# shiyao-li/NextBestPath

Hardware: AMD Instinct MI355X
Metric: exploration steps/s (+ NBP maps/s) at 256x256 (higher is better)
Workload: dtype f32

## Files before the change

### include/nbp_hip.h

```cpp
#ifndef NBP_HIP_H
#define NBP_HIP_H

#include <stddef.h>
#include <stdint.h>

#ifdef __cplusplus
extern "C" {
#endif

#define NBP_E_ARG      (-1)
#define NBP_E_WS       (-2)
#define NBP_E_SHAPE    (-3)

int nbp_abi_version(void);
int nbp_device_info(char* arch_host, int arch_len, int* cu_count_host);
int nbp_tuning_active(void);
int nbp_tuning_report(char* buf_host, int len);
int nbp_tile_kernel_symbol(int tile, char* buf_host, int len);

#define NBP_N_CONV 48

typedef struct nbp_weights nbp_weights;

size_t nbp_packed_weights_bytes(void);
// ... 47 lines not shown
int nbp_pack_conv_weight_split(const float* w_oihw, int N, int C, int ksize, const float* scale_or_null, int c_off,
                               int c_total, void* dst_planes, void* wamax_out, void* stream);
int nbp_amax_f32(const float* x, long long n, void* amax_inout, void* stream);
int nbp_pack_upconv_weight_split(const float* w_oihw, int N, int C, void* dst_planes, void* wamax_out, void* stream);
int nbp_upconv3x3_split_f32(const float* src, int C, int B, int H, int W, const void* planes_up, const void* wamax_up, int N,
                            const float* scale, const float* shift, int relu, float* out, const void* amax_in_or_null,
                            void* amax_out_or_null, int split_k, void* ws, size_t ws_bytes, void* stream);
size_t nbp_conv_split_workspace_bytes(int B, int H, int W, int N, int split_k);
size_t nbp_conv_split_planned_workspace_bytes(int B, int H, int W, int C, int N, int ups, int* split_k_out);
size_t nbp_conv_split_planned_workspace_bytes_k(int B, int H, int W, int C, int N, int ups, int split_k, int* split_k_out);
int nbp_conv3x3_split_f32(const float* src0, int C0, const float* src1, int C1, int ups, int B, int H, int W,
                          const void* w_planes, const void* wamax, int N, const float* scale, const float* shift, int relu,
                          float* out, const void* amax_in_or_null, void* amax_out_or_null, int split_k, void* ws,
                          size_t ws_bytes, void* stream);
size_t nbp_conv_first_wgrad_workspace_bytes(void);
int nbp_conv_first_wgrad_f32(const float* x_nchw, int B, int H, int W, const float* dy, float* dw, void* ws, size_t ws_bytes, void* stream);
int nbp_prepack_weights_split(const void* descs_dev, int n, void* wamax_words, void* stream);
int nbp_prepack_desc_bytes(void);
int nbp_pack_conv_weight_split_prezeroed(const float* w_oihw, int N, int C, int ksize, int c_total, void* dst_planes,
                                         void* wamax_zeroed, void* stream);
int nbp_pack_conv_weight_split_dgrad_known(const float* w_oihw, int N, int C, int c_total, void* dst_planes, const void* wamax_known,
                                           void* stream);
int nbp_pack_upconv_weight_split_dgrad(const float* w_oihw, int N, int C, void* dst_planes, void* wamax_out, void* stream);
size_t nbp_upconv_split_dgrad_workspace_bytes(int B, int H, int W, int N, int C);
int nbp_upconv3x3_split_dgrad_f32(const float* dy, int N, int B, int H, int W, const void* planes, const void* wamax, int C,
                                  const float* scale, const float* shift, float* dx, const void* amax_in, void* amax_out_or_null,
                                  void* ws, size_t ws_bytes, void* stream);
size_t nbp_upconv_wgrad_split_workspace_bytes(int B, int Hs, int Ws, int C, int N);
int nbp_upconv_wgrad_split_f32(const float* x, int C, int B, int Hs, int Ws, const float* dy, int N, float* dw,
                               const void* amax_x, const void* amax_y, void* ws, size_t ws_bytes, void* stream);
int nbp_conv1x1_split_f32(const float* src, int C, long long M, const void* w_planes, const void* wamax, int N,
                          const float* scale, const float* shift, int relu, float* out, const void* amax_in, void* stream);
int nbp_pack_conv1x1_weight_split_dgrad(const float* w_nc, int N, int C, void* dst_planes, void* wamax_out, void* stream);
int nbp_pack_conv_weight_split_dgrad(const float* w_oihw, int N, int C, int c_total, void* dst_planes, void* wamax_out, void* stream);

int nbp_conv_bn_part_rows(int B, int H, int W);
int nbp_conv3x3_split_bn_f32(const float* src0, int C0, const float* src1, int C1, int ups, int B, int H, int W,
                             const void* w_planes, const void* wamax, int N, const float* scale, const float* shift, int relu,
                             float* out, const void* amax_in_or_null, void* amax_out_or_null, int split_k, void* ws,
                             size_t ws_bytes, double* bn_part, int* bn_rows, void* stream);
int nbp_upconv3x3_split_bn_f32(const float* src, int C, int B, int H, int W, const void* planes_up, const void* wamax_up, int N,
                               const float* scale, const float* shift, int relu, float* out, const void* amax_in_or_null,
                               void* amax_out_or_null, int split_k, void* ws, size_t ws_bytes, double* bn_part, int* bn_rows,
                               void* stream);
int nbp_pack_conv_weight_split_h1(const float* w_oihw, int N, int C, int ksize, const float* scale_or_null, int c_off,
                                  int c_total, void* dst_planes, void* wamax_out, void* stream);
int nbp_pack_conv_weight_split_prezeroed_h1(const float* w_oihw, int N, int C, int ksize, int c_total, void* dst_planes,
                                            void* wamax_zeroed, void* stream);
int nbp_pack_conv_weight_split_dgrad_h1(const float* w_oihw, int N, int C, int c_total, void* dst_planes, void* wamax_out, void* stream);
int nbp_pack_conv_weight_split_dgrad_known_h1(const float* w_oihw, int N, int C, int c_total, void* dst_planes, const void* wamax_known,
                                              void* stream);
int nbp_pack_upconv_weight_split_h1(const float* w_oihw, int N, int C, void* dst_planes, void* wamax_out, void* stream);
int nbp_pack_upconv_weight_split_dgrad_h1(const float* w_oihw, int N, int C, void* dst_planes, void* wamax_out, void* stream);
int nbp_pack_conv1x1_weight_split_dgrad_h1(const float* w_nc, int N, int C, void* dst_planes, void* wamax_out, void* stream);
int nbp_prepack_weights_split_h1(const void* descs_dev, int n, void* wamax_words, void* stream);
int nbp_conv3x3_split_f32_h1(const float* src0, int C0, const float* src1, int C1, int ups, int B, int H, int W,
                             const void* w_planes, const void* wamax, int N, const float* scale, const float* shift, int relu,
                             float* out, const void* amax_in_or_null, void* amax_out_or_null, int split_k, void* ws,
                             size_t ws_bytes, void* stream);
int nbp_conv3x3_split_bn_f32_h1(const float* src0, int C0, const float* src1, int C1, int ups, int B, int H, int W,
                                const void* w_planes, const void* wamax, int N, const float* scale, const float* shift, int relu,
                                float* out, const void* amax_in_or_null, void* amax_out_or_null, int split_k, void* ws,
                                size_t ws_bytes, double* bn_part, int* bn_rows, void* stream);
int nbp_upconv3x3_split_f32_h1(const float* src, int C, int B, int H, int W, const void* planes_up, const void* wamax_up, int N,
                               const float* scale, const float* shift, int relu, float* out, const void* amax_in_or_null,
                               void* amax_out_or_null, int split_k, void* ws, size_t ws_bytes, void* stream);
// ... 352 lines not shown
```

### nextbestpath_amd/_lib.py

```python
from __future__ import annotations

import ctypes as C
import os
import threading

HERE = os.path.dirname(os.path.abspath(__file__))
LIB_PATH = os.path.join(HERE, "libnbp_hip.so")

_vp, _i, _ll, _f, _sz, _d = C.c_void_p, C.c_int, C.c_longlong, C.c_float, C.c_size_t, C.c_double

SIGNATURES = {
    "nbp_abi_version": (_i, []),
    "nbp_device_info": (_i, [C.c_char_p, _i, C.POINTER(_i)]),
    "nbp_tuning_active": (_i, []),
    "nbp_tuning_report": (_i, [C.c_char_p, _i]),
    "nbp_tile_kernel_symbol": (_i, [_i, C.c_char_p, _i]),
    "nbp_packed_weights_bytes": (_sz, []),
    "nbp_pack_weights": (_i, [C.POINTER(_vp), C.POINTER(_vp), C.POINTER(_vp), _vp, _sz, _vp, C.POINTER(_vp)]),
    "nbp_free_weights": (None, [_vp]),
    "nbp_forward_workspace_bytes": (_sz, [_i, _i]),
    "nbp_forward_f32": (_i, [_vp, _vp, _i, _i, _vp, _vp, _vp, _sz, _vp]),
    "nbp_forward_flops": (_d, [_i, _i]),
    "nbp_conv_igemm_f32": (_i, [_vp, _i, _vp, _i, _i, _i, _i, _i, _i, _vp, _i, _vp, _vp, _i, _vp, _i, _i, _vp,
                                _sz, _vp]),
# ... 87 lines not shown
SIGNATURES["nbp_packed_weights_bytes_bf16"] = SIGNATURES["nbp_packed_weights_bytes"]
SIGNATURES["nbp_pack_upconv_weight_bf16"] = (_i, [_vp, _i, _i, _vp, _vp])
SIGNATURES["nbp_forward_workspace_bytes_bf16"] = SIGNATURES["nbp_forward_workspace_bytes"]
SIGNATURES["nbp_forward_bf16"] = SIGNATURES["nbp_forward_f32"]
SIGNATURES["nbp_packed_weights_bytes_split"] = SIGNATURES["nbp_packed_weights_bytes"]
SIGNATURES["nbp_pack_weights_split"] = SIGNATURES["nbp_pack_weights"]
SIGNATURES["nbp_forward_workspace_bytes_split"] = SIGNATURES["nbp_forward_workspace_bytes"]
SIGNATURES["nbp_forward_split_f32"] = SIGNATURES["nbp_forward_f32"]
SIGNATURES["nbp_forward_timed_split_f32"] = SIGNATURES["nbp_forward_timed_f32"]
SIGNATURES["nbp_pack_conv_weight_split"] = (_i, [_vp, _i, _i, _i, _vp, _i, _i, _vp, _vp, _vp])
SIGNATURES["nbp_amax_f32"] = (_i, [_vp, _ll, _vp, _vp])
SIGNATURES["nbp_pack_upconv_weight_split"] = (_i, [_vp, _i, _i, _vp, _vp, _vp])
SIGNATURES["nbp_upconv3x3_split_f32"] = (_i, [_vp, _i, _i, _i, _i, _vp, _vp, _i, _vp, _vp, _i, _vp, _vp, _vp, _i, _vp, _sz, _vp])
SIGNATURES["nbp_conv_split_workspace_bytes"] = SIGNATURES["nbp_conv_igemm_workspace_bytes"]
SIGNATURES["nbp_conv_split_planned_workspace_bytes"] = (_sz, [_i, _i, _i, _i, _i, _i, _vp])
SIGNATURES["nbp_conv_split_planned_workspace_bytes_k"] = (_sz, [_i, _i, _i, _i, _i, _i, _i, _vp])
SIGNATURES["nbp_conv3x3_split_f32"] = (_i, [_vp, _i, _vp, _i, _i, _i, _i, _i, _vp, _vp, _i, _vp, _vp, _i, _vp, _vp, _vp, _i, _vp,
                                            _sz, _vp])
SIGNATURES["nbp_pack_upconv_weight_split_dgrad"] = (_i, [_vp, _i, _i, _vp, _vp, _vp])
SIGNATURES["nbp_upconv_split_dgrad_workspace_bytes"] = (_sz, [_i, _i, _i, _i, _i])
SIGNATURES["nbp_upconv3x3_split_dgrad_f32"] = (_i, [_vp, _i, _i, _i, _i, _vp, _vp, _i, _vp, _vp, _vp, _vp, _vp, _vp, _sz, _vp])
SIGNATURES["nbp_upconv_wgrad_split_workspace_bytes"] = (_sz, [_i, _i, _i, _i, _i])
SIGNATURES["nbp_upconv_wgrad_split_f32"] = (_i, [_vp, _i, _i, _i, _i, _vp, _i, _vp, _vp, _vp, _vp, _sz, _vp])
SIGNATURES["nbp_pack_conv_weight_split_prezeroed"] = (_i, [_vp, _i, _i, _i, _i, _vp, _vp, _vp])
SIGNATURES["nbp_pack_conv_weight_split_dgrad_known"] = (_i, [_vp, _i, _i, _i, _vp, _vp, _vp])
SIGNATURES["nbp_prepack_weights_split"] = (_i, [_vp, _i, _vp, _vp])
SIGNATURES["nbp_prepack_desc_bytes"] = (_i, [])
SIGNATURES["nbp_rowscale_amax_f32"] = (_i, [_vp, _vp, _ll, _i, _vp, _vp, _vp])
SIGNATURES["nbp_conv_first_linear_f32"] = (_i, [_vp, _i, _i, _i, _vp, _vp, _vp, _vp, _vp])
SIGNATURES["nbp_conv_first_wgrad_workspace_bytes"] = (_sz, [])
SIGNATURES["nbp_conv_first_wgrad_f32"] = (_i, [_vp, _i, _i, _i, _vp, _vp, _vp, _sz, _vp])
SIGNATURES["nbp_conv1x1_split_f32"] = (_i, [_vp, _i, _ll, _vp, _vp, _i, _vp, _vp, _i, _vp, _vp, _vp])
SIGNATURES["nbp_pack_conv1x1_weight_split_dgrad"] = (_i, [_vp, _i, _i, _vp, _vp, _vp])
SIGNATURES["nbp_pack_conv_weight_split_dgrad"] = (_i, [_vp, _i, _i, _i, _vp, _vp, _vp])
SIGNATURES["nbp_conv_bn_part_rows"] = (_i, [_i, _i, _i])
SIGNATURES["nbp_conv3x3_split_bn_f32"] = (_i, [_vp, _i, _vp, _i, _i, _i, _i, _i, _vp, _vp, _i, _vp, _vp, _i, _vp, _vp, _vp, _i, _vp,
                                               _sz, _vp, C.POINTER(_i), _vp])
SIGNATURES["nbp_upconv3x3_split_bn_f32"] = (_i, [_vp, _i, _i, _i, _i, _vp, _vp, _i, _vp, _vp, _i, _vp, _vp, _vp, _i, _vp, _sz, _vp,
                                                 C.POINTER(_i), _vp])
SIGNATURES["nbp_bn_train_forward_part4_f32"] = (_i, [_vp, _ll, _i, _vp, _vp, _f, _f, _vp, _vp, _i, _vp, _vp, _vp, _vp, _vp, _i, _vp, _i, _vp, _vp])
for _n in ("nbp_pack_conv_weight_split", "nbp_pack_conv_weight_split_prezeroed", "nbp_pack_conv_weight_split_dgrad",
           "nbp_pack_conv_weight_split_dgrad_known", "nbp_pack_upconv_weight_split", "nbp_pack_upconv_weight_split_dgrad",
           "nbp_pack_conv1x1_weight_split_dgrad", "nbp_prepack_weights_split", "nbp_conv3x3_split_f32", "nbp_conv3x3_split_bn_f32",
           "nbp_upconv3x3_split_f32", "nbp_upconv3x3_split_bn_f32", "nbp_upconv3x3_split_dgrad_f32", "nbp_conv1x1_split_f32",
           "nbp_upconv_wgrad_split_f32", "nbp_conv_wgrad_split_f32"):
    SIGNATURES[_n + "_h1"] = SIGNATURES[_n]
SIGNATURES["nbp_conv_igemm_bf16"] = SIGNATURES["nbp_conv_igemm_f32"]
SIGNATURES["nbp_conv_igemm_bf16_workspace_bytes"] = SIGNATURES["nbp_conv_igemm_workspace_bytes"]
SIGNATURES["nbp_pack_conv_weight_bf16"] = SIGNATURES["nbp_pack_conv_weight"]
SIGNATURES["nbp_f32_to_bf16"] = (_i, [_vp, _ll, _vp, _vp])
SIGNATURES["nbp_bf16_to_f32"] = (_i, [_vp, _ll, _vp, _vp])
_fpp, _ipp = C.POINTER(_f), C.POINTER(_i)
SIGNATURES["nbp_scene_fill_workspace_bytes"] = (_sz, [_fpp, _ipp, _i, _ll, _d])
SIGNATURES["nbp_scene_fill_cells_f32"] = (_i, [_vp, _ll, _vp, _fpp, _ipp, _i, _d, _i, C.c_uint, _vp, _vp, _vp, _sz, _vp])
SIGNATURES["nbp_scene_gather_f32"] = (_i, [_vp, _vp, _i, _i, _vp, _ll, _vp, _vp])
SIGNATURES["nbp_scene_coverage_workspace_bytes"] = (_sz, [_fpp, _ipp, _i, _d])
SIGNATURES["nbp_scene_coverage_f32"] = (_i, [_vp, _vp, _i, _vp, _vp, _i, _fpp, _ipp, _d, _vp, _vp, _sz, _vp])
SIGNATURES["nbp_coverage_plan_bytes"] = (_sz, [_fpp, _fpp, _f, _i])
SIGNATURES["nbp_coverage_plan_workspace_bytes"] = (_sz, [_fpp, _fpp, _f, _i])
SIGNATURES["nbp_coverage_plan_build_f32"] = (_i, [_vp, _i, _f, _fpp, _fpp, _vp, _sz, _vp, _sz, _vp])
SIGNATURES["nbp_coverage_count_planned_f32"] = (_i, [_vp, _i, _f, _fpp, _fpp, _vp, _ll, _vp, _ll, C.c_uint, C.c_uint, _vp, _vp,
                                                     _vp])
SIGNATURES["nbp_points_in_fov_u8"] = (_i, [_vp, _i, _fpp, _i, _i, _i, _f, _f, _vp, _vp, _vp])
SIGNATURES["nbp_sample_points_f32"] = (_i, [_vp, _ll, _vp, _ll, C.c_uint, _vp, _vp, _vp])
SIGNATURES["nbp_raster_rgb_workspace_bytes"] = (_sz, [_i, _i, _i, _i])
SIGNATURES["nbp_raster_rgbz_f32"] = (_i, [_vp, _i, _vp, _i, _vp, _fpp, _i, _i, _i, _f, _f, _f, _f, _vp, _vp, _vp, _sz, _vp])
# ... 137 lines not shown
```

### nextbestpath_amd/csrc/nbp_internal.h

```cpp
#pragma once
#include "common.h"

typedef unsigned short bf16_t;

enum { NBP_TILE_AUTO = 0, NBP_TILE_128x128 = 1, NBP_TILE_256x64 = 2, NBP_TILE_256x32 = 3, NBP_TILE_128x64 = 4,
       NBP_TILE_64x128 = 5,
       NBP_TILE_HALO_128 = 6, NBP_TILE_HALO_64 = 7,
       NBP_TILE_HALO4_128 = 8, NBP_TILE_HALO4_64 = 9,
       NBP_TILE_SPLIT_HALO_64 = 10, NBP_TILE_SPLIT_UP = 11,
       NBP_TILE_HALO_UP_128 = 12, NBP_TILE_HALO_UP_64 = 13,
       NBP_TILE_RESERVED_14 = 14,
       NBP_TILE_SPLIT_HALO_R8 = 15, NBP_TILE_SPLIT_UP_R8 = 16,
       NBP_TILE_SPLIT_UP_DGRAD = 17,
       NBP_TILE_SPLIT_HALO_128 = 18,
       NBP_TILE_SPLIT_GATE = 19 };
struct TileInfo { int bm, bn; };
struct ConvPlan { int tile; int split_k; int chunks_per_split; };

struct IgemmArgs {
    const float* src0;
    const float* src1;
    int C0, C1;
    int cc0;
    int ups;
// ... 22 lines not shown
    float* g_out;
    int xcd_remap;
};
struct ConvOperands { const float* src0; const float* src1; const float* wpk; const float* scale; const float* shift; float* out; };
ConvPlan nbp_plan_conv(long long M, int N, int chunks_total, int tile, int split_k, int groups, int H = 0, int W = 0,
                       int ksize = 0);
int nbp_conv_igemm_launch_g(const ConvOperands& o, const ConvOperands* o2, int C0, int C1, int ups, int B, int H, int W,
                            int ksize, int N, int relu, int split_k, int tile, void* ws, size_t ws_bytes, hipStream_t st);

struct ConvOperandsSplit {
    const float* src0; const float* src1; const void* planes; const float* scale; const float* shift; float* out;
    const unsigned* amax0; const unsigned* amax1; const unsigned* wamax; unsigned* amax_out;
    const void* planes_up; const unsigned* wamax_up;
    const float* psi0 = nullptr;
};
ConvPlan nbp_plan_conv_split(long long M, int N, int chunks_total, int split_k, int groups, int H, int W, int ksize, int ups = 0);
int nbp_pack_upconv_weight_split_launch(const float* w_oihw, int N, int C, void* dst, unsigned* wamax_out, hipStream_t st, int one = 0);
struct ConvHead { const float* w; const float* scale; const float* shift; float* out; };
int nbp_conv_split_launch_g(const ConvOperandsSplit& o, const ConvOperandsSplit* o2, int C0, int C1, int ups, int B, int H, int W,
                            int ksize, int N, int relu, int split_k, void* ws, size_t ws_bytes, hipStream_t st,
                            float* const* pool_out = nullptr, int* pooled = nullptr, const struct ConvHead* head = nullptr,
                            int* headed = nullptr, double* bn_part = nullptr, int* bn_rows = nullptr, int one = 0);
int nbp_pack_conv_weight_split_launch(const float* w_oihw, int N, int C, int ksize, const float* scale_or_null, int c_off,
                                      int c_total, void* dst, unsigned* wamax_out, hipStream_t st, int one = 0);
int nbp_amax_launch(const float* x, long long n, unsigned* amax_inout, hipStream_t st);
int nbp_wgrad_split_launch(const float* src0, int C0, const float* src1, int C1, int ups, int B, int H, int W, const float* dy, int N,
                           int n_tiles, int splits, unsigned* amax3, const unsigned* amax0_in, const unsigned* amax1_in,
                           const unsigned* amaxy_in, float* part, hipStream_t st);
int nbp_pack_gate_weight_split_launch(const float* wg, const float* scale_g, const float* wx, const float* scale_x, int N, int C,
                                      void* dst, unsigned* wamax_out, hipStream_t st);
struct GatePsi { const float* wpsi[2]; const float* st[2]; float* gated[2]; unsigned* gated_amax[2] = {nullptr, nullptr};
                 int psi_only = 0; };
int nbp_gate1x1_split_launch_g(const ConvOperandsSplit& o, const ConvOperandsSplit* o2, int C, long long M, int N, int relu,
                               hipStream_t st, const GatePsi* psi = nullptr, int* fused = nullptr);
int nbp_conv_first_amax_launch(const float* x_nchw, int B, int H, int W, const float* w_oihw, const float* scale, const float* shift,
                               float* out_nhwc, unsigned* amax_out, int* did_amax, hipStream_t st);

struct ConvOperandsH { const bf16_t* src0; const bf16_t* src1; const bf16_t* wpk; const float* scale; const float* shift; bf16_t* out;
                       const bf16_t* wpk_up; };
ConvPlan nbp_plan_conv_bf16(long long M, int N, int chunks_total, int tile, int split_k, int groups, int H = 0, int W = 0,
                            int ksize = 0, int ups = 0);
int nbp_pack_upconv_weight_bf16_launch(const float* w_oihw, int N, int C, bf16_t* dst, hipStream_t st);
struct GatePsiH { const float* wpsi[2]; const float* st[2]; bf16_t* gated[2]; };
int nbp_conv_igemm_bf16_launch_g(const ConvOperandsH& o, const ConvOperandsH* o2, int C0, int C1, int ups, int B, int H,
                                 int W, int ksize, int N, int relu, int split_k, int tile, void* ws, size_t ws_bytes,
                                 hipStream_t st, bf16_t* const* pool_out = nullptr, int* pooled = nullptr,
                                 const struct ConvHead* head = nullptr, int* headed = nullptr, const GatePsiH* psi = nullptr,
                                 int* psi_fused = nullptr);
int nbp_conv_first_bf16_launch(const float* x_nchw, int B, int H, int W, const float* w_oihw, const float* scale,
                               const float* shift, bf16_t* out_nhwc, hipStream_t st);
int nbp_maxpool2_bf16_launch(const bf16_t* in, int B, int H, int W, int C, bf16_t* out, hipStream_t st);
int nbp_psi_gate_bf16_launch(const bf16_t* q, int F, const float* w_psi, const float* s_t2, const bf16_t* x, int C,
                             long long M, bf16_t* out, hipStream_t st);
int nbp_final_1x1_bf16_launch(const bf16_t* in, int B, int H, int W, int C, const float* w_oc, int n_out,
                              const float* scale, const float* shift, int sigmoid, float* out_nchw, hipStream_t st);
```

### nextbestpath_amd/csrc/nbp_split.hip

```cpp
#include "common.h"
#include "nbp_internal.h"
#include <cstdlib>

namespace {

typedef _Float16 f16x8 __attribute__((ext_vector_type(8)));
typedef _Float16 f16x2 __attribute__((ext_vector_type(2)));
typedef unsigned u32x4 __attribute__((ext_vector_type(4)));
typedef unsigned u32x2 __attribute__((ext_vector_type(2)));
typedef __attribute__((address_space(3))) void* lds_ptr_t;

constexpr int SPLIT_EXP = 14;
__host__ __device__ inline int amax_exponent(unsigned bits) {
    if (!bits) return SPLIT_EXP;
    int e = (int)((bits >> 23) & 255u) - 127;
    return e < -100 ? -100 : (e > 100 ? 100 : e);
}
__host__ __device__ inline float pow2f(int e) {
    union { unsigned u; float f; } v;
    v.u = (unsigned)(127 + e) << 23;
    return v.f;
}

__device__ __forceinline__ void split_pair(float x0, float x1, unsigned& h, unsigned& l) {
// ... 673 lines not shown
            f32x4 v[4];
#pragma unroll
            for (int u = 0; u < 4; ++u) { const int i = i0 + 64 * u; if (i < total && i < lim) v[u] = x4[i]; }
#pragma unroll
            for (int u = 0; u < 4; ++u) {
                const int i = i0 + 64 * u;
                if (i < total && i < lim) {
                    const float ps = psil[i / C4];
                    const f32x4 g = v[u] * ps;
                    if (!a.psi_only) g4[i] = g;
                    gmx = fmaxf(fmaxf(gmx, fmaxf(fabsf(g[0]), fabsf(g[1]))), fmaxf(fabsf(g[2]), fabsf(g[3])));
                }
            }
        }
        if (a.gated_amax[blockIdx.z]) wave_amax(gmx, a.gated_amax[blockIdx.z]);
    } else {
#pragma unroll
    for (int j = 0; j < TN; ++j) {
        const int n = n0 + j * 32 + (lane & 31);
        const float sc = o.scale[n], sh = o.shift[n];
#pragma unroll
        for (int r = 0; r < 16; ++r) {
            const long long mm = mw + (r & 3) + 8 * (r >> 2) + 4 * khalf;
            if (mm < a.M) {
                float v = ldexpf(acc[j][r], einv) * sc + sh;
                if (a.relu) v = fmaxf(v, 0.f);
                o.out[mm * a.N + n] = v;
            }
        }
    }
    }
}

struct WgradSplitArgs {
    const float* src0; const float* src1;
    int C0, C1, ups, H, W, Hs, Ws;
    const float* dy; int N;
    unsigned bytes0, bytes1, bytesy;
    int co_tiles, n_tiles, splits;
    const unsigned* amax0; const unsigned* amax1; const unsigned* amaxy;
    float* part;
};
typedef short s16x4 __attribute__((ext_vector_type(4)));
typedef __attribute__((address_space(3))) s16x4* lds_s16x4_t;

__device__ __forceinline__ f16x8 tr_frag(const char* p) {
    const s16x4 a = __builtin_amdgcn_ds_read_tr16_b64_v4i16((lds_s16x4_t)(p));
    const s16x4 b = __builtin_amdgcn_ds_read_tr16_b64_v4i16((lds_s16x4_t)(p + 256));
    typedef short s16x8 __attribute__((ext_vector_type(8)));
    const s16x8 v = {a[0], a[1], a[2], a[3], b[0], b[1], b[2], b[3]};
    return __builtin_bit_cast(f16x8, v);
}

template <int TW, bool ONE = false>
__global__ __launch_bounds__(256, 2) void wgrad_split_kernel(WgradSplitArgs a) {
    constexpr int TR = 64 / TW, HW_ = TW + 2, HP = (TR + 2) * HW_;
    constexpr int NX = (HP * 16 + 255) / 256;
    constexpr int XPL = HP * 64, YPL = 64 * 64;
    constexpr int XB = (ONE ? 2 : 4) * XPL;
    extern __shared__ __attribute__((aligned(16))) char wl[];
    const int tid = threadIdx.x, lane = tid & 63, wave = tid >> 6;
    const int wi = wave >> 1, wj = wave & 1, kh = lane >> 5, ln = lane & 31;
    const int ci0 = (blockIdx.x / a.co_tiles) * 64, co0 = (blockIdx.x % a.co_tiles) * 64;
    const int Ctot = a.C0 + a.C1;
    const bool first = ci0 < a.C0;
    const int Cs = first ? a.C0 : a.C1;
// ... 952 lines not shown
int nbp_pack_upconv_weight_split_launch(const float* w_oihw, int N, int C, void* dst, unsigned* wamax_out, hipStream_t st, int one) {
    NBP_RETURN_IF(!w_oihw || !dst || !wamax_out, NBP_E_ARG);
    NBP_RETURN_IF(N < 1 || C < 16 || C % 16, NBP_E_SHAPE);
    hipError_t e = hipMemsetAsync(wamax_out, 0, sizeof(unsigned), st);
    if (e != hipSuccess) return (int)e;
    const long long NC = (long long)N * C;
    const int grid = nbp_ew_grid(NC, 256);
    if (one) {
        pack_upconv_h2_kernel<true><<<min(grid, 256), 256, 0, st>>>(w_oihw, N, C, wamax_out, nullptr);
        pack_upconv_h2_kernel<true><<<grid, 256, 0, st>>>(w_oihw, N, C, wamax_out, (unsigned short*)dst);
    } else {
        pack_upconv_h2_kernel<<<min(grid, 256), 256, 0, st>>>(w_oihw, N, C, wamax_out, nullptr);
        pack_upconv_h2_kernel<<<grid, 256, 0, st>>>(w_oihw, N, C, wamax_out, (unsigned short*)dst);
    }
    return nbp_launch_status();
}

int nbp_pack_gate_weight_split_launch(const float* wg, const float* scale_g, const float* wx, const float* scale_x, int N, int C,
                                      void* dst, unsigned* wamax_out, hipStream_t st) {
    NBP_RETURN_IF(!wg || !wx || !dst || !wamax_out, NBP_E_ARG);
    NBP_RETURN_IF(N < 32 || N % 32 || C < 32 || C % 32, NBP_E_SHAPE);
    hipError_t e = hipMemsetAsync(wamax_out, 0, sizeof(unsigned), st);
    if (e != hipSuccess) return (int)e;
    const long long total = (long long)N * C;
    const int grid = min(nbp_ew_grid(total, 256), 256);
    amax_kernel<<<grid, 256, 0, st>>>(wg, total, scale_g, C, wamax_out, 1u);
    amax_kernel<<<grid, 256, 0, st>>>(wx, total, scale_x, C, wamax_out, 1u);
    pack_conv_weight_h2_kernel<<<nbp_ew_grid(total, 256), 256, 0, st>>>(wg, N, C, 1, scale_g, 0, wamax_out, (unsigned short*)dst);
    pack_conv_weight_h2_kernel<<<nbp_ew_grid(total, 256), 256, 0, st>>>(wx, N, C, 1, scale_x, C, wamax_out, (unsigned short*)dst);
    return nbp_launch_status();
}

int nbp_gate1x1_split_launch_g(const ConvOperandsSplit& o, const ConvOperandsSplit* o2, int C, long long M, int N, int relu,
                               hipStream_t st, const GatePsi* psi, int* fused) {
    const int groups = o2 ? 2 : 1;
    NBP_RETURN_IF(!o.src0 || !o.src1 || !o.planes || !o.scale || !o.shift || !o.out || !o.amax0 || !o.amax1 || !o.wamax, NBP_E_ARG);
    NBP_RETURN_IF(o2 && (!o2->src0 || !o2->src1 || !o2->planes || !o2->out || !o2->amax0 || !o2->amax1 || !o2->wamax), NBP_E_ARG);
    NBP_RETURN_IF(C < 64 || C % 64 || N < 32 || N % 32 || M < 1, NBP_E_SHAPE);
    const long long b0 = M * C * 4, bw = 2ll * C * N * 4;
    NBP_RETURN_IF(b0 >= (1ll << 31) || bw >= (1ll << 31), NBP_E_SHAPE);
    GateArgs a;
    for (int g = 0; g < 2; ++g) {
        const ConvOperandsSplit& s = (g && o2) ? *o2 : o;
        a.g[g] = SplitOps{s.src0, s.src1, s.planes, s.scale, s.shift, s.out, s.amax0, s.amax1, s.wamax, nullptr, nullptr, nullptr, {nullptr, nullptr}, nullptr};
        const int gi = g < groups ? g : 0;
        a.wpsi[g] = psi ? psi->wpsi[gi] : nullptr; a.st[g] = psi ? psi->st[gi] : nullptr; a.gated[g] = psi ? psi->gated[gi] : nullptr;
        a.gated_amax[g] = psi ? psi->gated_amax[gi] : nullptr;
    }
    a.psi_only = psi ? psi->psi_only : 0;
    a.C = C; a.C1 = C; a.N = N; a.relu = relu; a.M = M; a.bytes0 = (unsigned)b0; a.bytesw = (unsigned)bw; a.groups = groups;
    int bn = N % 128 == 0 ? 128 : (N % 64 == 0 ? 64 : 32);
    static const int allow_psi = nbp_tune_int("NBP_GATE_PSI", 1);
    const bool psi_wants_128 = allow_psi && psi && N == 128 && psi->wpsi[0] && psi->st[0] && psi->gated[0];
    if (bn == 128 && nbp_cdiv(M, 128) * (N / 128) * groups < 512 && !psi_wants_128) bn = 64;
    const bool with_psi = allow_psi && psi && bn == N && psi->wpsi[0] && psi->st[0] && psi->gated[0] &&
                          (groups == 1 || (psi->wpsi[1] && psi->st[1] && psi->gated[1]));
    if (fused) *fused = with_psi;
    dim3 grid((unsigned)nbp_cdiv(M, 128), (unsigned)(N / bn), (unsigned)groups);
    const size_t smem = 2 * (size_t)8 * bn * 16;
    {
        char nm[64];
        snprintf(nm, sizeof(nm), "gate1x1_h2_kernel<false, %d, %s>", bn / 32, with_psi ? "true" : "false");
        nbp_note_kernel_symbol(NBP_TILE_SPLIT_GATE, nm);
    }
    if (with_psi) {
        if (bn == 128) gate1x1_h2_kernel<false, 4, true><<<grid, 256, smem, st>>>(a);
        else if (bn == 64) gate1x1_h2_kernel<false, 2, true><<<grid, 256, smem, st>>>(a);
        else gate1x1_h2_kernel<false, 1, true><<<grid, 256, smem, st>>>(a);
    } else if (bn == 128) gate1x1_h2_kernel<false, 4, false><<<grid, 256, smem, st>>>(a);
    else if (bn == 64) gate1x1_h2_kernel<false, 2, false><<<grid, 256, smem, st>>>(a);
    else gate1x1_h2_kernel<false, 1, false><<<grid, 256, smem, st>>>(a);
    return nbp_launch_status();
}

int nbp_upconv_dgrad_split_launch(const float* dy, int N, int B, int H, int W, const void* planes, const unsigned* wamax,
                                  const unsigned* amax_in, int C, const float* scale, const float* shift, float* out, unsigned* amax_out,
                                  int split_k, void* ws, size_t ws_bytes, hipStream_t st, int one = 0) {
    NBP_RETURN_IF(!dy || !planes || !wamax || !amax_in || !scale || !shift || !out, NBP_E_ARG);
    NBP_RETURN_IF(B < 1 || N < 16 || N % 16 || C < 64 || C % 64, NBP_E_SHAPE);
    const int tw = split_tile_width(H, W, C, 3);
    NBP_RETURN_IF(!tw, NBP_E_SHAPE);
    SplitArgs a;
    for (int g = 0; g < 2; ++g)
        a.g[g] = SplitOps{dy, nullptr, planes, scale, shift, out, amax_in, nullptr, wamax, amax_out, nullptr, nullptr, {nullptr, nullptr}, nullptr, nullptr};
    a.C0 = N; a.C1 = 0; a.ups = 0; a.H = H; a.W = W; a.Hs = 2 * H; a.Ws = 2 * W; a.N = C; a.relu = 0; a.groups = 1;
    a.M = (long long)B * H * W;
    const long long b0 = (long long)B * 4 * H * W * N * 4, bw = 64ll * N * C;
    NBP_RETURN_IF(b0 >= (1ll << 31) || bw >= (1ll << 31), NBP_E_SHAPE);
    a.bytes0 = (unsigned)b0; a.bytes1 = (unsigned)b0; a.bytesw = (unsigned)bw;
    a.chunks_total = 4 * (N / 16);
// ... 377 lines not shown
    int sk = 1;
    while (blocks * sk < 256 && chunks / (sk * 2) >= 4 && sk < 16) sk *= 2;
    return 256 + (sk > 1 ? (size_t)sk * M * C * sizeof(float) : 0);
}
extern "C" int nbp_upconv3x3_split_dgrad_f32(const float* dy, int N, int B, int H, int W, const void* planes, const void* wamax, int C,
                                             const float* scale, const float* shift, float* dx, const void* amax_in, void* amax_out_or_null,
                                             void* ws, size_t ws_bytes, void* stream) {
    NBP_ENTER();
    return nbp_upconv_dgrad_split_launch(dy, N, B, H, W, planes, (const unsigned*)wamax, (const unsigned*)amax_in, C, scale, shift, dx,
                                         (unsigned*)amax_out_or_null, 0, ws ? (char*)ws + 256 : nullptr, ws_bytes >= 256 ? ws_bytes - 256 : 0,
                                         (hipStream_t)stream);
}
extern "C" int nbp_upconv3x3_split_dgrad_f32_h1(const float* dy, int N, int B, int H, int W, const void* planes, const void* wamax, int C,
                                                const float* scale, const float* shift, float* dx, const void* amax_in, void* amax_out_or_null,
                                                void* ws, size_t ws_bytes, void* stream) {
    NBP_ENTER();
    return nbp_upconv_dgrad_split_launch(dy, N, B, H, W, planes, (const unsigned*)wamax, (const unsigned*)amax_in, C, scale, shift, dx,
                                         (unsigned*)amax_out_or_null, 0, ws ? (char*)ws + 256 : nullptr, ws_bytes >= 256 ? ws_bytes - 256 : 0,
                                         (hipStream_t)stream, 1);
}

extern "C" int nbp_conv1x1_split_f32(const float* src, int C, long long M, const void* w_planes, const void* wamax, int N,
                                     const float* scale, const float* shift, int relu, float* out, const void* amax_in, void* stream) {
    NBP_ENTER();
    return nbp_conv1x1_split_launch(src, C, M, w_planes, (const unsigned*)wamax, (const unsigned*)amax_in, N, scale, shift, relu, out,
                                    (hipStream_t)stream);
}
extern "C" int nbp_conv1x1_split_f32_h1(const float* src, int C, long long M, const void* w_planes, const void* wamax, int N,
                                        const float* scale, const float* shift, int relu, float* out, const void* amax_in, void* stream) {
    NBP_ENTER();
    return nbp_conv1x1_split_launch(src, C, M, w_planes, (const unsigned*)wamax, (const unsigned*)amax_in, N, scale, shift, relu, out,
                                    (hipStream_t)stream, 1);
}
template <bool ONE>
static int pack_conv1x1_weight_split_dgrad_impl(const float* w_nc, int N, int C, void* dst_planes, void* wamax_out, void* stream) {
    NBP_RETURN_IF(!w_nc || !dst_planes || !wamax_out, NBP_E_ARG);
    NBP_RETURN_IF(N < 32 || N % 32 || C < 32 || C % 32, NBP_E_SHAPE);
    hipStream_t st = (hipStream_t)stream;
    const long long total = (long long)N * C;
    hipError_t e = hipMemsetAsync(wamax_out, 0, sizeof(unsigned), st);
    if (e != hipSuccess) return (int)e;
    amax_kernel<<<min(nbp_ew_grid(total, 256), 256), 256, 0, st>>>(w_nc, total, nullptr, C, (unsigned*)wamax_out, 1u);
    pack_conv_weight_h2_kernel<ONE><<<nbp_ew_grid(total, 256), 256, 0, st>>>(w_nc, C, N, 1, nullptr, 0, (const unsigned*)wamax_out,
                                                                            (unsigned short*)dst_planes, 1);
    return nbp_launch_status();
}
extern "C" int nbp_pack_conv1x1_weight_split_dgrad(const float* w_nc, int N, int C, void* dst_planes, void* wamax_out, void* stream) {
    NBP_ENTER();
    return pack_conv1x1_weight_split_dgrad_impl<false>(w_nc, N, C, dst_planes, wamax_out, stream);
}
extern "C" int nbp_pack_conv1x1_weight_split_dgrad_h1(const float* w_nc, int N, int C, void* dst_planes, void* wamax_out, void* stream) {
    NBP_ENTER();
    return pack_conv1x1_weight_split_dgrad_impl<true>(w_nc, N, C, dst_planes, wamax_out, stream);
}

extern "C" int nbp_pack_upconv_weight_split(const float* w_oihw, int N, int C, void* dst_planes, void* wamax_out, void* stream) {
    NBP_ENTER();
    return nbp_pack_upconv_weight_split_launch(w_oihw, N, C, dst_planes, (unsigned*)wamax_out, (hipStream_t)stream);
}
extern "C" int nbp_pack_upconv_weight_split_h1(const float* w_oihw, int N, int C, void* dst_planes, void* wamax_out, void* stream) {
    NBP_ENTER();
    return nbp_pack_upconv_weight_split_launch(w_oihw, N, C, dst_planes, (unsigned*)wamax_out, (hipStream_t)stream, 1);
}
extern "C" int nbp_pack_upconv_weight_split_dgrad_h1(const float* w_oihw, int N, int C, void* dst_planes, void* wamax_out, void* stream) {
    NBP_ENTER();
    return pack_upconv_weight_split_dgrad_impl<true>(w_oihw, N, C, dst_planes, wamax_out, stream);
// ... 62 lines not shown
```

Measured before the change: 2317.

## Add persistent pipelined gate 1x1 kernel with resident weights and prefetched activations

Adds a persistent-grid variant of the fused attention-gate 1x1 conv plus psi kernel for the small shapes (N=32/C=64 and N=64/C=128). It loads all weight planes into LDS once per block, then walks tiles while prefetching activation loads several stages ahead in registers to hide memory latency. The grid defaults to twice the CU count and can be overridden by an env knob or argument. It also exposes new C entry points for this gate kernel and its weight packing. The cost is higher register and LDS use, which caps occupancy.

```diff
diff --git a/include/nbp_hip.h b/include/nbp_hip.h
--- a/include/nbp_hip.h
+++ b/include/nbp_hip.h
@@ -103,6 +103,12 @@
 int nbp_conv1x1_split_f32(const float* src, int C, long long M, const void* w_planes, const void* wamax, int N,
                           const float* scale, const float* shift, int relu, float* out, const void* amax_in, void* stream);
 int nbp_pack_conv1x1_weight_split_dgrad(const float* w_nc, int N, int C, void* dst_planes, void* wamax_out, void* stream);
+int nbp_gate1x1_split_f32(const float* g, const float* x, int C, long long M, const void* w_planes, const void* wamax, int N,
+                          const float* scale, const float* shift, const void* amax_g, const void* amax_x, const float* w_psi,
+                          const float* st_psi, float* q_out, float* gated_out, void* gated_amax, int psi_only, int pipe_grid,
+                          int* fused_host, void* stream);
+int nbp_pack_gate_weight_split(const float* wg, const float* scale_g, const float* wx, const float* scale_x, int N, int C,
+                               void* dst_planes, void* wamax_out, void* stream);
 int nbp_pack_conv_weight_split_dgrad(const float* w_oihw, int N, int C, int c_total, void* dst_planes, void* wamax_out, void* stream);
 
 int nbp_conv_bn_part_rows(int B, int H, int W);
diff --git a/nextbestpath_amd/_lib.py b/nextbestpath_amd/_lib.py
--- a/nextbestpath_amd/_lib.py
+++ b/nextbestpath_amd/_lib.py
@@ -143,6 +143,9 @@
 SIGNATURES["nbp_conv_first_wgrad_f32"] = (_i, [_vp, _i, _i, _i, _vp, _vp, _vp, _sz, _vp])
 SIGNATURES["nbp_conv1x1_split_f32"] = (_i, [_vp, _i, _ll, _vp, _vp, _i, _vp, _vp, _i, _vp, _vp, _vp])
 SIGNATURES["nbp_pack_conv1x1_weight_split_dgrad"] = (_i, [_vp, _i, _i, _vp, _vp, _vp])
+SIGNATURES["nbp_gate1x1_split_f32"] = (_i, [_vp, _vp, _i, _ll, _vp, _vp, _i, _vp, _vp, _vp, _vp, _vp, _vp, _vp, _vp, _vp, _i, _i,
+                                            C.POINTER(_i), _vp])
+SIGNATURES["nbp_pack_gate_weight_split"] = (_i, [_vp, _vp, _vp, _vp, _i, _i, _vp, _vp, _vp])
 SIGNATURES["nbp_pack_conv_weight_split_dgrad"] = (_i, [_vp, _i, _i, _i, _vp, _vp, _vp])
 SIGNATURES["nbp_conv_bn_part_rows"] = (_i, [_i, _i, _i])
 SIGNATURES["nbp_conv3x3_split_bn_f32"] = (_i, [_vp, _i, _vp, _i, _i, _i, _i, _i, _vp, _vp, _i, _vp, _vp, _i, _vp, _vp, _vp, _i, _vp,
diff --git a/nextbestpath_amd/csrc/nbp_internal.h b/nextbestpath_amd/csrc/nbp_internal.h
--- a/nextbestpath_amd/csrc/nbp_internal.h
+++ b/nextbestpath_amd/csrc/nbp_internal.h
@@ -78,7 +78,7 @@
 struct GatePsi { const float* wpsi[2]; const float* st[2]; float* gated[2]; unsigned* gated_amax[2] = {nullptr, nullptr};
                  int psi_only = 0; };
 int nbp_gate1x1_split_launch_g(const ConvOperandsSplit& o, const ConvOperandsSplit* o2, int C, long long M, int N, int relu,
-                               hipStream_t st, const GatePsi* psi = nullptr, int* fused = nullptr);
+                               hipStream_t st, const GatePsi* psi = nullptr, int* fused = nullptr, int pipe_grid = -1);
 int nbp_conv_first_amax_launch(const float* x_nchw, int B, int H, int W, const float* w_oihw, const float* scale, const float* shift,
                                float* out_nhwc, unsigned* amax_out, int* did_amax, hipStream_t st);
 
diff --git a/nextbestpath_amd/csrc/nbp_split.hip b/nextbestpath_amd/csrc/nbp_split.hip
--- a/nextbestpath_amd/csrc/nbp_split.hip
+++ b/nextbestpath_amd/csrc/nbp_split.hip
@@ -729,6 +729,176 @@
     }
 }
 
+template <int TN>
+__global__ __launch_bounds__(256, 2) void gate1x1_h2_pipe_kernel(GateArgs a, int ntiles) {
+    const SplitOps& o = a.g[blockIdx.z];
+    constexpr int BN = TN * 32;
+    constexpr int S = TN * 4;
+    constexpr int D = 8;
+    constexpr int WST = 8 * BN * 16;
+    constexpr int WI = WST / 1024;
+    extern __shared__ __attribute__((aligned(16))) char wbuf[];
+    const int tid = threadIdx.x, lane = tid & 63, wave = tid >> 6;
+    const int khalf = lane >> 5;
+    const int G = gridDim.x;
+    const int my = ((int)blockIdx.x < ntiles) ? (ntiles - (int)blockIdx.x + G - 1) / G : 0;
+    const unsigned ma0 = read_amax(o.amax0), ma1 = read_amax(o.amax1);
+    const int ea = amax_exponent(ma0 > ma1 ? ma0 : ma1), ew = amax_exponent(*o.wamax);
+    const float sa = pow2f(SPLIT_EXP - ea);
+    const int einv = ea + ew - 2 * SPLIT_EXP;
+    const __amdgpu_buffer_rsrc_t rs0 = __builtin_amdgcn_make_buffer_rsrc(const_cast<float*>(o.src0), 0, a.bytes0, 0x00020000);
+    const __amdgpu_buffer_rsrc_t rs1 = __builtin_amdgcn_make_buffer_rsrc(const_cast<float*>(o.src1), 0, a.bytes0, 0x00020000);
+    const __amdgpu_buffer_rsrc_t rsw = __builtin_amdgcn_make_buffer_rsrc(const_cast<void*>(o.planes), 0, a.bytesw, 0x00020000);
+    constexpr unsigned OOB = 0x80000000u;
+
+#pragma unroll
+    for (int st = 0; st < S; ++st)
+#pragma unroll
+        for (int k = 0; k < (WI + 3) / 4; ++k) {
+            const int q = wave + 4 * k;
+            if (q < WI) {
+                constexpr int PER = BN / 64 > 0 ? BN / 64 : 1;
+                const int r8 = BN >= 64 ? q / PER : q * 2 + (lane >> 5), nb = BN >= 64 ? q - (q / PER) * PER : 0;
+                const int row = BN >= 64 ? nb * 64 + lane : (lane & 31);
+                const int ks = r8 >> 2, r4 = r8 & 3;
+                const unsigned woff = (unsigned)((((long long)(2 * st + ks) * 4 + r4) * a.N + row) * 16);
+                __builtin_amdgcn_raw_ptr_buffer_load_lds(rsw, (lds_ptr_t)(wbuf + st * WST + q * 1024), 16, woff, 0, 0, 0);
+            }
+        }
+
+    u32x4 xr[D][2][2];
+    auto load_x = [&](int i, int s, int slot) {
+        const long long m = ((long long)blockIdx.x + (long long)i * G) * 128 + wave * 32 + (lane & 31);
+        const bool ok = i < my && m < a.M;
+        const bool first = s < S / 2;
+        const unsigned cb = (unsigned)((first ? s : s - S / 2) * 32 + khalf * 8) * 4u;
+        const unsigned prow = (unsigned)(m * a.C) * 4u;
+#pragma unroll
+        for (int ks = 0; ks < 2; ++ks)
+#pragma unroll
+            for (int h = 0; h < 2; ++h) {
+                const unsigned off = ok ? prow + cb + ks * 64 + h * 16 : OOB;
+                xr[slot][ks][h] = first ? __builtin_amdgcn_raw_buffer_load_b128(rs0, off, 0, 0) : __builtin_amdgcn_raw_buffer_load_b128(rs1, off, 0, 0);
+            }
+    };
+#pragma unroll
+    for (int q = 0; q < D - 1; ++q) load_x(q / S, q % S, q);
+
+    float sc[TN], sh[TN], wp[TN];
+#pragma unroll
+    for (int j = 0; j < TN; ++j) {
+        const int n = j * 32 + (lane & 31);
+        sc[j] = o.scale[n]; sh[j] = o.shift[n]; wp[j] = a.wpsi[blockIdx.z][n];
+    }
+    const float st0 = a.st[blockIdx.z][0], st1 = a.st[blockIdx.z][1];
+    float* psil = reinterpret_cast<float*>(wbuf + S * WST) + wave * 32;
+    constexpr int C4 = 2 * BN / 4, total = 32 * C4;
+    float gmx = 0.f;
+
+    asm volatile("s_waitcnt vmcnt(0)" ::: "memory");
+    __syncthreads();
+
+    f32x16 acc[TN];
+    for (int i0 = 0; i0 < my; i0 += D / S) {
+#pragma unroll
+        for (int u = 0; u < D; ++u) {
+            const int i = i0 + u / S;
+            const int s = u % S;
+            load_x(i0 + (u + D - 1) / S, (u + D - 1) % S, (u + D - 1) % D);
+            if (i < my) {
+                if (s == 0)
+#pragma unroll
+                    for (int j = 0; j < TN; ++j)
+#pragma unroll
+                        for (int r = 0; r < 16; ++r) acc[j][r] = 0.f;
+                const char* Bt = wbuf + s * WST + khalf * (BN * 16) + (lane & 31) * 16;
+#pragma unroll
+                for (int ks = 0; ks < 2; ++ks) {
+                    const f32x4 v0 = __builtin_bit_cast(f32x4, xr[u][ks][0]), v1 = __builtin_bit_cast(f32x4, xr[u][ks][1]);
+                    unsigned h0, l0, h1, l1, h2, l2, h3, l3;
+                    split_pair(v0[0] * sa, v0[1] * sa, h0, l0); split_pair(v0[2] * sa, v0[3] * sa, h1, l1);
+                    split_pair(v1[0] * sa, v1[1] * sa, h2, l2); split_pair(v1[2] * sa, v1[3] * sa, h3, l3);
+                    const u32x4 xh = u32x4{h0, h1, h2, h3}, xl = u32x4{l0, l1, l2, l3};
+#pragma unroll
+                    for (int j = 0; j < TN; ++j) {
+                        const u32x4 wh = *reinterpret_cast<const u32x4*>(Bt + ((ks * 2 + 0) * 2) * (BN * 16) + j * 512);
+                        const u32x4 wl = *reinterpret_cast<const u32x4*>(Bt + ((ks * 2 + 1) * 2) * (BN * 16) + j * 512);
+                        acc[j] = __builtin_amdgcn_mfma_f32_32x32x16_f16(__builtin_bit_cast(f16x8, xl), __builtin_bit_cast(f16x8, wh), acc[j], 0, 0, 0);
+                        acc[j] = __builtin_amdgcn_mfma_f32_32x32x16_f16(__builtin_bit_cast(f16x8, xh), __builtin_bit_cast(f16x8, wl), acc[j], 0, 0, 0);
+                        acc[j] = __builtin_amdgcn_mfma_f32_32x32x16_f16(__builtin_bit_cast(f16x8, xh), __builtin_bit_cast(f16x8, wh), acc[j], 0, 0, 0);
+                    }
+                }
+                if (s == S - 1) {
+                    const long long mw = ((long long)blockIdx.x + (long long)i * G) * 128 + wave * 32;
+                    float p[16];
+#pragma unroll
+                    for (int r = 0; r < 16; ++r) p[r] = 0.f;
+#pragma unroll
+                    for (int j = 0; j < TN; ++j)
+#pragma unroll
+                        for (int r = 0; r < 16; ++r) {
+                            float v = ldexpf(acc[j][r], einv) * sc[j] + sh[j];
+                            if (a.relu) v = fmaxf(v, 0.f);
+                            p[r] = fmaf(v, wp[j], p[r]);
+                        }
+                    float p8[8], p4[4], p2[2];
+                    {
+                        const bool up = lane & 16;
+#pragma unroll
+                        for (int k = 0; k < 8; ++k) p8[k] = (up ? p[8 + k] : p[k]) + __shfl_xor(up ? p[k] : p[8 + k], 16);
+                    }
+                    {
+                        const bool up = lane & 8;
+#pragma unroll
+                        for (int k = 0; k < 4; ++k) p4[k] = (up ? p8[4 + k] : p8[k]) + __shfl_xor(up ? p8[k] : p8[4 + k], 8);
+                    }
+                    {
+                        const bool up = lane & 4;
+#pragma unroll
+                        for (int k = 0; k < 2; ++k) p2[k] = (up ? p4[2 + k] : p4[k]) + __shfl_xor(up ? p4[k] : p4[2 + k], 4);
+                    }
+                    float dot;
+                    {
+                        const bool up = lane & 2;
+                        dot = (up ? p2[1] : p2[0]) + __shfl_xor(up ? p2[0] : p2[1], 2);
+                    }
+                    dot += __shfl_xor(dot, 1);
+                    const float z = dot * st0 + st1;
+                    const float psi = 1.f / (1.f + expf(-z));
+                    const int r = (lane & 31) >> 1;
+                    if (!(lane & 1)) {
+                        const int pix = (r & 3) + 8 * (r >> 2) + 4 * khalf;
+                        psil[pix] = psi;
+                        if (a.psi_only && mw + pix < a.M) a.gated[blockIdx.z][mw + pix] = psi;
+                    }
+                    asm volatile("s_waitcnt lgkmcnt(0)" ::: "memory");
+                    f32x4* g4 = reinterpret_cast<f32x4*>(a.gated[blockIdx.z]) + mw * C4;
+                    const long long lim = (a.M - mw) * C4;
+                    const unsigned xbase = (unsigned)(mw * (2 * BN)) * 4u;
+#pragma unroll 1
+                    for (int k0 = lane; k0 < total; k0 += 256) {
+                        u32x4 v[4];
+#pragma unroll
+                        for (int w = 0; w < 4; ++w) {
+                            const int k = k0 + 64 * w;
+                            v[w] = __builtin_amdgcn_raw_buffer_load_b128(rs1, k < lim ? xbase + (unsigned)k * 16u : OOB, 0, 0);
+                        }
+#pragma unroll
+                        for (int w = 0; w < 4; ++w) {
+                            const int k = k0 + 64 * w;
+                            const float ps = psil[k / C4];
+                            const f32x4 g = __builtin_bit_cast(f32x4, v[w]) * ps;
+                            if (!a.psi_only && k < lim) g4[k] = g;
+                            gmx = fmaxf(fmaxf(gmx, fmaxf(fabsf(g[0]), fabsf(g[1]))), fmaxf(fabsf(g[2]), fabsf(g[3])));
+                        }
+                    }
+                }
+            }
+        }
+    }
+    if (a.gated_amax[blockIdx.z]) wave_amax(gmx, a.gated_amax[blockIdx.z]);
+}
+
 struct WgradSplitArgs {
     const float* src0; const float* src1;
     int C0, C1, ups, H, W, Hs, Ws;
@@ -1747,7 +1917,7 @@
 }
 
 int nbp_gate1x1_split_launch_g(const ConvOperandsSplit& o, const ConvOperandsSplit* o2, int C, long long M, int N, int relu,
-                               hipStream_t st, const GatePsi* psi, int* fused) {
+                               hipStream_t st, const GatePsi* psi, int* fused, int pipe_grid) {
     const int groups = o2 ? 2 : 1;
     NBP_RETURN_IF(!o.src0 || !o.src1 || !o.planes || !o.scale || !o.shift || !o.out || !o.amax0 || !o.amax1 || !o.wamax, NBP_E_ARG);
     NBP_RETURN_IF(o2 && (!o2->src0 || !o2->src1 || !o2->planes || !o2->out || !o2->amax0 || !o2->amax1 || !o2->wamax), NBP_E_ARG);
@@ -1771,6 +1941,35 @@
     const bool with_psi = allow_psi && psi && bn == N && psi->wpsi[0] && psi->st[0] && psi->gated[0] &&
                           (groups == 1 || (psi->wpsi[1] && psi->st[1] && psi->gated[1]));
     if (fused) *fused = with_psi;
+    {
+        static const int knob = nbp_tune_int("NBP_GATE_PIPE_GRID", -1);
+        static const int dflt = [] {
+            int dev = 0, cus = 0;
+            if (hipGetDevice(&dev) != hipSuccess || hipDeviceGetAttribute(&cus, hipDeviceAttributeMultiprocessorCount, dev) != hipSuccess || cus < 1) cus = 256;
+            return 2 * cus;
+        }();
+        const int want = pipe_grid >= 0 ? pipe_grid : (knob >= 0 ? knob : dflt);
+        const long long tiles = nbp_cdiv(M, 128);
+        const int gx = want / groups;
+        if (with_psi && want > 0 && gx >= 1 && ((N == 32 && C == 64) || (N == 64 && C == 128)) && tiles >= gx && tiles < (1ll << 31)) {
+            if (fused) *fused = 2;
+            char nm[64];
+            snprintf(nm, sizeof(nm), "gate1x1_h2_pipe_kernel<%d>", N / 32);
+            nbp_note_kernel_symbol(NBP_TILE_SPLIT_GATE, nm);
+            dim3 grid((unsigned)gx, 1u, (unsigned)groups);
+            const size_t smem = (size_t)(N / 8) * 8 * N * 16 + 512;
+            static bool attr_set = false;
+            if (!attr_set) {
+                const hipError_t e = hipFuncSetAttribute(reinterpret_cast<const void*>(&gate1x1_h2_pipe_kernel<2>),
+                                                         hipFuncAttributeMaxDynamicSharedMemorySize, 8 * 8 * 64 * 16 + 512);
+                if (e != hipSuccess) return (int)e;
+                attr_set = true;
+            }
+            if (N == 32) gate1x1_h2_pipe_kernel<1><<<grid, 256, smem, st>>>(a, (int)tiles);
+            else gate1x1_h2_pipe_kernel<2><<<grid, 256, smem, st>>>(a, (int)tiles);
+            return nbp_launch_status();
+        }
+    }
     dim3 grid((unsigned)nbp_cdiv(M, 128), (unsigned)(N / bn), (unsigned)groups);
     const size_t smem = 2 * (size_t)8 * bn * 16;
     {
@@ -2214,6 +2413,27 @@
     return nbp_conv1x1_split_launch(src, C, M, w_planes, (const unsigned*)wamax, (const unsigned*)amax_in, N, scale, shift, relu, out,
                                     (hipStream_t)stream, 1);
 }
+extern "C" int nbp_gate1x1_split_f32(const float* g, const float* x, int C, long long M, const void* w_planes, const void* wamax, int N,
+                                     const float* scale, const float* shift, const void* amax_g, const void* amax_x, const float* w_psi,
+                                     const float* st_psi, float* q_out, float* gated_out, void* gated_amax, int psi_only, int pipe_grid,
+                                     int* fused_host, void* stream) {
+    NBP_ENTER();
+    NBP_RETURN_IF(w_psi && (!st_psi || !gated_out), NBP_E_ARG);
+    const ConvOperandsSplit o{g, x, w_planes, scale, shift, q_out, (const unsigned*)amax_g, (const unsigned*)amax_x, (const unsigned*)wamax,
+                              nullptr, nullptr, nullptr};
+    GatePsi psi;
+    for (int k = 0; k < 2; ++k) { psi.wpsi[k] = w_psi; psi.st[k] = st_psi; psi.gated[k] = gated_out; psi.gated_amax[k] = (unsigned*)gated_amax; }
+    psi.psi_only = psi_only;
+    int fused = 0;
+    const int rc = nbp_gate1x1_split_launch_g(o, nullptr, C, M, N, 1, (hipStream_t)stream, w_psi ? &psi : nullptr, &fused, pipe_grid);
+    if (fused_host) *fused_host = fused;
+    return rc;
+}
+extern "C" int nbp_pack_gate_weight_split(const float* wg, const float* scale_g, const float* wx, const float* scale_x, int N, int C,
+                                          void* dst_planes, void* wamax_out, void* stream) {
+    NBP_ENTER();
+    return nbp_pack_gate_weight_split_launch(wg, scale_g, wx, scale_x, N, C, dst_planes, (unsigned*)wamax_out, (hipStream_t)stream);
+}
 template <bool ONE>
 static int pack_conv1x1_weight_split_dgrad_impl(const float* w_nc, int N, int C, void* dst_planes, void* wamax_out, void* stream) {
     NBP_RETURN_IF(!w_nc || !dst_planes || !wamax_out, NBP_E_ARG);
```

Result: no change. 2327 (median of 6 runs) (+0.5%).
